# sergcpp/Ray

Measured on AMD Instinct MI355X. Metric: Msamples/sec (W*H*spp/time), higher is better.
Workload: dtype f32

## Files before the change

ray_amd/csrc/bvh_hooks.h:

```cpp
#pragma once

#include <string>
#include <vector>

#include "bvh4_build.h"
#include "lbvh.h"

namespace rayhip_bvh_hooks {

inline bool check_lbvh_args(const float *boxes, const uint32_t *groups, const uint32_t n_prims, const uint32_t n_groups, const uint32_t leaf_max,
                            std::string &why) {
    if (leaf_max < 1 || leaf_max > 8) {
        why = "leaf_max must be 1..8";
        return false;
    }
    if (n_prims >= 0x10000000u) {
        why = "too many primitives for a leaf word";
        return false;
    }
    if (n_prims && (!boxes || !groups)) {
        why = "null input";
        return false;
    }
    for (uint32_t p = 0; p < n_prims; ++p) {
        if (groups[p] >= n_groups) {
            why = "a group id is out of range";
            return false;
        }
    }
// ... 74 lines not shown
    }
    if (res.nodes.size() > n_nodes) {
        why = "more wide nodes than BVH2 nodes";
        return 1;
    }
    std::copy(res.nodes.begin(), res.nodes.end(), out_wide);
    std::copy(res.blas_root4.begin(), res.blas_root4.end(), out_roots4);
    *out_count = uint32_t(res.nodes.size());
    return 0;
}

RT_HD void test_node_item(const rt::Bvh4Node *wide, const uint32_t node, const float *o, const float *d, const float t, uint32_t *out_ref,
                          uint32_t *out_n_hit, float *out_dist) {
    const rt::f3 inv_d = rt::safe_invert(rt::f3{d[0], d[1], d[2]});
    uint32_t ref[4], n_hit;
    float dist[4];
    rt::bvh4_test_node(wide, node, rt::f3{o[0], o[1], o[2]}, inv_d, t, ref, n_hit, dist);
    for (int c = 0; c < 4; ++c) {
        out_ref[c] = ref[c], out_dist[c] = dist[c];
    }
    *out_n_hit = n_hit;
}

inline bool check_items(const uint32_t *node_index, const uint32_t n_items, const uint32_t n_wide, std::string &why) {
    for (uint32_t i = 0; i < n_items; ++i) {
        if (node_index[i] >= n_wide) {
            why = "an item names a node outside the array";
            return false;
        }
    }
    return true;
}

}
```

ray_amd/csrc/kernels_closest_refill.hip.h:

```cpp
#pragma once

#ifndef RT_REFILL_MIN
#define RT_REFILL_MIN 40
#endif
#ifndef RT_REFILL_MIN_WAVES
#define RT_REFILL_MIN_WAVES 6
#endif
#ifndef RT_REFILL_VOTE_NUM
#define RT_REFILL_VOTE_NUM 1
#define RT_REFILL_VOTE_DEN 1
#endif
#ifndef RT_REFILL_RUN
#define RT_REFILL_RUN 1
#endif
#ifndef RT_REFILL_MIN_DIRECT
#define RT_REFILL_MIN_DIRECT 40
#endif
template <int WIDE, int MIN_WAIT = RT_REFILL_MIN, bool DIRECT = false>
__global__ void __launch_bounds__(WAVE, RT_REFILL_MIN_WAVES) k_trace_closest_refill(const SceneView sc, const TraceParams tp, const RaySoA rays,
                                                               const HitSoA hits, const RayQueue queue, const int init_hits,
                                                               uint32_t *__restrict__ stack_spill, const Layering layers,
                                                               uint32_t *__restrict__ work ) {
    __shared__ uint32_t lds_stack[LDS_STACK_DEPTH * WAVE];
    const uint32_t lane = threadIdx.x;
#ifdef RT_PROFILE_TRACE
    if (threadIdx.x < 32) {
        s_prof_acc[threadIdx.x] = 0;
    }
    if (threadIdx.x == 0) {
        s_prof_last = __builtin_readcyclecounter();
    }
#endif
    LdsStack st;
    st.lane_base = &lds_stack[lane];
    st.spill_base = stack_spill + size_t(blockIdx.x) * size_t(STACK_SPILL_DEPTH * WAVE) + lane;
    st.size = 0;

    enum : uint32_t { IDLE = 0, TLAS = 1, BLAS = 2 };
#ifdef RT_PROFILE_TRACE
    uint32_t st_a = 0, st_b = 0, st_iter = 0, st_serv = 0, st_serv_lanes = 0, st_tlas = 0;
#endif
    uint32_t lvl = IDLE, slot = 0, cur = BVH4_SENTINEL, tos = BVH4_SENTINEL, size = 0, mi_index = 0, ray_flags = 0;
    uint32_t cur_bits = 0, tos_bits = 0, tri_base = 0, l0 = 0, l1 = 0, oct_inv = 0;
    bool res = false;
    f3 ro = {0.0f, 0.0f, 0.0f}, rd = {0.0f, 0.0f, 1.0f};
    f3 o = ro, d = rd, inv_d = rd;
    Hit h = make_hit();
    float t_val = 0.0f;
    uint32_t pool_slot = 0, pool_left = 0;
    ChunkWalk walk(queue.live_chunks(), work, RT_REFILL_RUN);

    auto begin_round = [&]() {
        t_val = h.t;
        res = false;
        size = 0;
        if (DIRECT) {
            tos = BVH4_SENTINEL;
            if ((sc.direct.ray_visibility & ray_flags) != 0) {
                o = transform_point(ro, sc.direct.inv_xform);
                d = transform_direction(rd, sc.direct.inv_xform);
                inv_d = safe_invert(d);
                st.write_at(size++, BVH4_SENTINEL);
                cur = sc.direct.root;
                lvl = (cur == BVH4_SENTINEL) ? TLAS : BLAS;
            } else {
                cur = BVH4_SENTINEL;
                lvl = TLAS;
            }
            return;
        }
        st.write_at(size++, BVH4_SENTINEL);
        tos = BVH4_SENTINEL;
        cur = tp.root_index;
        lvl = TLAS;
    };
    auto pop = [&]() {
        cur = tos;
        tos = st.read_at(--size);
    };
    auto leave_blas = [&]() {
        if (WIDE == 8) {
            if (lvl == BLAS && cur == BVH8_SENTINEL) {
                lvl = TLAS;
                cur = st.read_at(--size);
                tos = st.read_at(--size);
            }
        } else if (lvl == BLAS && cur == BVH4_SENTINEL) {
            lvl = TLAS;
            if (!DIRECT) {
                pop();
            }
        }
    };
    auto pop8 = [&]() {
        cur = tos, cur_bits = tos_bits;
        size -= 2;
        st.read2_at(size, tos, tos_bits);
    };

    uint32_t n_dead = 0;
    for (;;) {
        for (;;) {
            const bool in_blas = (lvl == BLAS);
            const bool leaf_word = (WIDE == 8 ? (l0 | l1) != 0u : (cur & BVH2_PRIM_COUNT_BITS) != 0);
            const unsigned long long m_blas = __builtin_amdgcn_ballot_w64(in_blas), m_leaf_word = __builtin_amdgcn_ballot_w64(leaf_word);
            const bool at_leaf = in_blas && leaf_word;
            const bool at_node = in_blas && !leaf_word;
            const int n_node = uniform_count(m_blas & ~m_leaf_word), n_leaf = uniform_count(m_blas & m_leaf_word);
            const int n_out = WAVE - n_node - n_leaf - int(n_dead);
#ifdef RT_PROFILE_TRACE
            st_a += n_node, st_b += n_leaf, st_iter += 1;
#endif
            if (n_node + n_leaf == 0 || n_out >= MIN_WAIT) {
                break;
            }
            if (n_node * RT_REFILL_VOTE_DEN >= n_leaf * RT_REFILL_VOTE_NUM) {
                if (at_node) {
                    if (WIDE == 8) {
                        const uint32_t node = bvh8_take_child(cur, cur_bits, oct_inv);
                        if ((cur_bits >> 8) != 0u) {
                            st.write2_at(size, tos, tos_bits);
                            size += 2;
                            tos = cur, tos_bits = cur_bits;
                        }
                        Bvh8Visit v;
                        bvh8_test_node(sc.nodes8, node, o, inv_d, h.t, oct_inv, v);
                        cur = v.child_base, cur_bits = v.bits, tri_base = v.tri_base, l0 = v.leaf[0], l1 = v.leaf[1];
                        if ((cur_bits >> 8) == 0u && (l0 | l1) == 0u) {
                            pop8();
                        }
                    } else {
                        bvh4_visit(sc.nodes4, o, inv_d, h.t, st, cur, tos, size);
                    }
                    leave_blas();
                }
                RT_PROF_T(19)
            } else {
                if (at_leaf) {
                    const uint32_t word = WIDE == 8 ? bvh8_take_leaf(tri_base, l0, l1) : cur;
                    const int tri_start = int(word & BVH2_PRIM_INDEX_BITS), tri_end = int(tri_start + ((word & BVH2_PRIM_COUNT_BITS) >> 29) + 1);
                    const bool hit = intersect_tris_closest(o, d, tri_table(sc), tri_start, tri_end, DIRECT ? int(sc.direct.mi) : int(mi_index), h);
                    res |= hit;
                    if (WIDE == 8) {
                        if ((l0 | l1) == 0u && (cur_bits >> 8) == 0u) {
                            pop8();
                        }
                    } else {
                        pop();
                    }
                    leave_blas();
                }
                RT_PROF_T(26)
            }
        }

#ifdef RT_PROFILE_TRACE
        st_serv += 1, st_serv_lanes += uint32_t(__popcll(__ballot(lvl != BLAS))) - n_dead;
#endif
        {
            const bool in_fin = (lvl == TLAS) && (cur == BVH4_SENTINEL);
            if (in_fin) {
                if (h.prim_index < 0) {
                    h.prim_index = -int(sc.tri_indices[-h.prim_index - 1]) - 1;
                } else {
                    h.prim_index = int(sc.tri_indices[h.prim_index]);
                }
                bool again = false;
                if (res && !hit_side_is_solid(sc, h)) {
                    const float4 cc = rays.c_cs[slot];
                    const uint2 xd = rays.xy_depth[slot];
                    Ray r;
                    r.c = {cc.x, cc.y, cc.z};
                    r.cone_spread = cc.w;
                    r.xy = xd.x, r.depth = xd.y;
                    const uint32_t xy_virtual = r.xy, layer = xy_layer(xy_virtual, layers);
                    TraceParams tpl = tp;
                    if (layer != 0) {
                        tpl.iteration = tp.iteration + int(layer);
                        tpl.rand_seed = layer_rand_seed(tpl.iteration);
                    }
// ... 141 lines not shown
```

ray_amd/csrc/kernels_shadow.hip.h:

```cpp
#pragma once

template <bool COUNT, int WIDE, int MINW = RT_TRACE_MIN_WAVES>
__global__ void __launch_bounds__(WAVE, MINW) k_trace_shadow(const SceneView sc, const TraceParams tp, const ShadowSoA shadow,
                                                      const RayQueue queue, const float limit,
                                                      const int img_w, float4 *__restrict__ temp_buf,
                                                      float4 *__restrict__ out_rc,
                                                      uint32_t *__restrict__ stack_spill,
                                                      unsigned long long *__restrict__ counters, const Layering layers) {
    __shared__ uint32_t lds_stack[LDS_STACK_DEPTH * WAVE];
    const uint32_t lane = threadIdx.x;
    const uint32_t n_live_chunks = queue.live_chunks();
    ChunkWalk walk(n_live_chunks);
    for (uint32_t c; walk.next(c);) {
        uint32_t stripe, slot0, n_live;
        if (!queue.chunk(c, stripe, slot0, n_live) || lane >= n_live) {
            continue;
        }
        const uint32_t i = slot0 + lane;
        const ShadowRay r = load_shadow(shadow, i);
        LdsStack st;
        st.lane_base = &lds_stack[lane];
        st.spill_base = stack_spill + size_t(blockIdx.x) * size_t(STACK_SPILL_DEPTH * WAVE) + lane;
        st.size = 0;
        TravCount tc = {0, 0, 0, 0, 0};
// ... 42 lines not shown
    st.size = 0;

    enum : uint32_t { IDLE = 0, TLAS = 1, BLAS = 2 };
    uint32_t lvl = IDLE, slot = 0, cur = BVH4_SENTINEL, tos = BVH4_SENTINEL, size = 0, mi_index = 0, crossed = 0;
    bool solid = false;
    f3 ro = {0.0f, 0.0f, 0.0f}, rd = {0.0f, 0.0f, 1.0f}, o = ro, d = rd, inv_d = rd;
    float dist = 0.0f;
    Hit h = make_hit();
    uint32_t pool_slot = 0, pool_left = 0;
    ChunkWalk walk(queue.live_chunks(), work, RT_SHADOW_RUN);

    auto begin_segment = [&]() {
        h = make_hit();
        h.t = dist;
        size = 0;
        if (DIRECT) {
            const bool walk_it = (sc.direct.ray_visibility & (1u << RAY_TYPE_SHADOW)) != 0 && sc.direct.root != BVH4_SENTINEL;
            o = transform_point(ro, sc.direct.inv_xform);
            d = transform_direction(rd, sc.direct.inv_xform);
            inv_d = safe_invert(d);
            st.write_at(size++, BVH4_SENTINEL);
            tos = BVH4_SENTINEL;
            cur = walk_it ? sc.direct.root : BVH4_SENTINEL;
            lvl = walk_it ? BLAS : TLAS;
            return;
        }
        st.write_at(size++, BVH4_SENTINEL);
        tos = BVH4_SENTINEL;
        cur = tp.root_index;
        lvl = TLAS;
    };
    auto pop = [&]() {
        cur = tos;
        tos = st.read_at(--size);
    };
    auto leave_blas = [&]() {
        if (lvl == BLAS && cur == BVH4_SENTINEL) {
            lvl = TLAS;
            if (!DIRECT) {
                pop();
            }
        }
    };
    auto deliver = [&](const f3 rc, const uint32_t xy_virtual) {
        if (out_rc) {
            out_rc[slot] = mkfloat4(rc.x, rc.y, rc.z, 0.0f);
        } else {
            add_shadow_pixel(rc, limit, xy_virtual, img_w, temp_buf);
        }
    };

    uint32_t n_dead = 0;
    for (;;) {
        for (;;) {
            const bool in_blas = (lvl == BLAS);
            const bool leaf_word = (cur & BVH2_PRIM_COUNT_BITS) != 0;
            const unsigned long long m_blas = __builtin_amdgcn_ballot_w64(in_blas), m_leaf_word = __builtin_amdgcn_ballot_w64(leaf_word);
            const bool at_leaf = in_blas && leaf_word;
            const bool at_node = in_blas && !leaf_word;
            const int n_node = uniform_count(m_blas & ~m_leaf_word), n_leaf = uniform_count(m_blas & m_leaf_word);
            const int n_out = WAVE - n_node - n_leaf - int(n_dead);
            if (n_node + n_leaf == 0 || n_out >= MIN_WAIT) {
                break;
            }
            if (n_node >= n_leaf) {
                if (at_node) {
                    bvh4_visit(sc.nodes4, o, inv_d, h.t, st, cur, tos, size);
                    leave_blas();
                }
            } else if (at_leaf) {
                const int tri_start = int(cur & BVH2_PRIM_INDEX_BITS), tri_end = int(tri_start + ((cur & BVH2_PRIM_COUNT_BITS) >> 29) + 1);
                bool stop = false;
                if (intersect_tris_any(o, d, tri_table(sc), sc.tri_materials, sc.tri_indices, tri_start, tri_end, DIRECT ? int(sc.direct.mi) : int(mi_index), h)) {
                    const bool is_backfacing = h.prim_index < 0;
                    const uint32_t prim = is_backfacing ? uint32_t(-h.prim_index - 1) : uint32_t(h.prim_index);
                    if (sc.all_solid != 0u) {
                        stop = true;
                    } else {
                        const rayhip_tri_mat_data md = sc.tri_materials[sc.tri_indices[prim]];
                        stop = (!is_backfacing && (md.front_mi & MATERIAL_SOLID_BIT)) || (is_backfacing && (md.back_mi & MATERIAL_SOLID_BIT));
                    }
                }
                if (stop) {
                    solid = true;
                    lvl = TLAS;
                    cur = BVH4_SENTINEL;
                } else {
                    pop();
                    leave_blas();
                }
            }
        }

        {
            const bool in_fin = (lvl == TLAS) && (cur == BVH4_SENTINEL);
            if (in_fin) {
                const uint32_t depth_word = float_as_uint(shadow.o_depth[slot].w);
                const float4 cx = shadow.c_xy[slot];
                const uint32_t xy_virtual = float_as_uint(cx.w);
                f3 rc = {cx.x, cx.y, cx.z};
                const bool over = (get_transp_depth(depth_word) + int(crossed)) > tp.max_transp_depth;
                if (solid || over) {
                    rc = {0.0f, 0.0f, 0.0f};
                }
                bool again = false;
                if (!solid && !over && h.v >= 0.0f) {
                    if (h.prim_index < 0) {
                        h.prim_index = -int(sc.tri_indices[-h.prim_index - 1]) - 1;
// ... 123 lines not shown
```

ray_amd/csrc/rayhip_hooks.hip.h:

```cpp
#pragma once


int rayhip_k_generate_primary_rays(rayhip_ctx *c, const rayhip_camera *cam, const int rect[4], int iteration,
                                   rayhip_ray *out_rays, rayhip_hit *out_hits, int *out_count) {
    if (use_device(c)) {
        return 1;
    }
    if (!c->w || !c->pmj.p || !c->filter_table.p) {
        return fail("k_generate_primary_rays needs resize + upload_static + set_filter_table first");
    }
    hipStream_t s = c->stream;
    const RayGenTiling tiling = make_raygen_tiling(c->w, c->h, rect[2], rect[3], c->shard);
    const size_t nslots = size_t(tiling.tiles) * 64u;
    if (c->clear_queues(1, s)) {
        return fail("queue counter clear failed");
    }
    const RayGenParams rg = make_raygen_params(*cam, c->w, c->h, rect, iteration, c->shard);
    k_raygen<<<grid_for(c, nslots, 256), 256, 0, s>>>(rg, c->sc.pmj, c->filter_table.as<float>(), c->px.required_samples,
                                                      c->rays[0], c->hits, c->ray_queue(0, nslots, 1), single_layer(c->w, c->h), tiling);
    HIP_TRY(hipGetLastError());
    uint32_t n = 0;
    HIP_TRY(hipMemcpyAsync(&n, c->ray_count(0), 4, hipMemcpyDeviceToHost, s));
    HIP_TRY(hipStreamSynchronize(s));
    HostRays hr;
// ... 261 lines not shown
    return 0;
}

__global__ void __launch_bounds__(256) k_bvh4_test_nodes(const Bvh4Node *__restrict__ wide, const uint32_t *__restrict__ node_index,
                                                        const float *__restrict__ ray_o, const float *__restrict__ ray_d,
                                                        const float *__restrict__ ray_t, const uint32_t n_items, uint32_t *__restrict__ out_ref,
                                                        uint32_t *__restrict__ out_n_hit, float *__restrict__ out_dist) {
    const uint32_t i = blockIdx.x * blockDim.x + threadIdx.x;
    if (i < n_items) {
        rayhip_bvh_hooks::test_node_item(wide, node_index[i], ray_o + size_t(i) * 3, ray_d + size_t(i) * 3, ray_t[i], out_ref + size_t(i) * 4,
                                         out_n_hit + i, out_dist + size_t(i) * 4);
    }
}

int rayhip_k_bvh4_test_nodes(rayhip_ctx *c, const void *wide, uint32_t n_wide, const uint32_t *node_index, const float *ray_o, const float *ray_d,
                             const float *ray_t, uint32_t n_items, uint32_t *out_ref, uint32_t *out_n_hit, float *out_dist) {
    if (use_device(c)) {
        return 1;
    }
    if (n_items == 0) {
        return 0;
    }
    std::string why;
    if (!rayhip_bvh_hooks::check_items(node_index, n_items, n_wide, why)) {
        return fail("k_bvh4_test_nodes: %s", why.c_str());
    }
    hipStream_t s = c->stream;
    const size_t n = n_items;
    DevBuf d_wide, d_idx, d_o, d_d, d_t, d_ref, d_hit, d_dist;
    if (d_wide.alloc(size_t(n_wide) * sizeof(Bvh4Node)) || d_idx.alloc(n * 4) || d_o.alloc(n * 12) || d_d.alloc(n * 12) || d_t.alloc(n * 4) ||
        d_ref.alloc(n * 16) || d_hit.alloc(n * 4) || d_dist.alloc(n * 16)) {
        return 1;
    }
    HIP_TRY(hipMemcpyAsync(d_wide.p, wide, size_t(n_wide) * sizeof(Bvh4Node), hipMemcpyHostToDevice, s));
    HIP_TRY(hipMemcpyAsync(d_idx.p, node_index, n * 4, hipMemcpyHostToDevice, s));
    HIP_TRY(hipMemcpyAsync(d_o.p, ray_o, n * 12, hipMemcpyHostToDevice, s));
    HIP_TRY(hipMemcpyAsync(d_d.p, ray_d, n * 12, hipMemcpyHostToDevice, s));
    HIP_TRY(hipMemcpyAsync(d_t.p, ray_t, n * 4, hipMemcpyHostToDevice, s));
    k_bvh4_test_nodes<<<(n_items + 255) / 256, 256, 0, s>>>(d_wide.as<Bvh4Node>(), d_idx.as<uint32_t>(), d_o.as<float>(), d_d.as<float>(),
                                                            d_t.as<float>(), n_items, d_ref.as<uint32_t>(), d_hit.as<uint32_t>(), d_dist.as<float>());
    HIP_TRY(hipGetLastError());
    HIP_TRY(hipMemcpyAsync(out_ref, d_ref.p, n * 16, hipMemcpyDeviceToHost, s));
    HIP_TRY(hipMemcpyAsync(out_n_hit, d_hit.p, n * 4, hipMemcpyDeviceToHost, s));
    HIP_TRY(hipMemcpyAsync(out_dist, d_dist.p, n * 16, hipMemcpyDeviceToHost, s));
    HIP_TRY(hipStreamSynchronize(s));
    d_wide.release(), d_idx.release(), d_o.release(), d_d.release(), d_t.release(), d_ref.release(), d_hit.release(), d_dist.release();
    return 0;
// ... 19 lines not shown
```

ray_amd/csrc/rayhip_upload.hip.h:

```cpp
#pragma once

static int upload_sky(rayhip_ctx *c, const rayhip_scene_desc *d) {
    c->sky_view = SkyView{};
    if (!(d->env.sky_map_spread_angle > 0.0f) || d->sky_count == 0) {
        return 0;
    }
    if (upload(c, c->sky_desc, d->sky, sizeof(rayhip_sky)) ||
        upload(c, c->sky_transmittance_lut, d->sky_transmittance_lut, size_t(d->sky_transmittance_lut_count) * sizeof(float)) ||
        upload(c, c->sky_multiscatter_lut, d->sky_multiscatter_lut, size_t(d->sky_multiscatter_lut_count) * sizeof(float)) ||
        upload(c, c->sky_dir_lights, d->sky_dir_lights, size_t(d->sky_dir_lights_count) * sizeof(uint32_t)) ||
        upload(c, c->sky_weather, d->sky_weather_tex, d->sky_weather_tex_count) || upload(c, c->sky_noise3d, d->sky_noise3d_tex, d->sky_noise3d_tex_count) ||
        upload(c, c->sky_curl, d->sky_curl_tex, d->sky_curl_tex_count) || upload(c, c->sky_moon, d->sky_moon_tex, d->sky_moon_tex_count) ||
        upload(c, c->sky_cirrus, d->sky_cirrus_tex, d->sky_cirrus_tex_count)) {
        return 1;
    }
    HIP_TRY(hipStreamSynchronize(c->stream));
    SkyView &v = c->sky_view;
    v.desc = c->sky_desc.as<rayhip_sky>();
    v.transmittance_lut = c->sky_transmittance_lut.as<float>(), v.multiscatter_lut = c->sky_multiscatter_lut.as<float>();
    v.dir_lights = c->sky_dir_lights.as<uint32_t>(), v.dir_lights_count = d->sky_dir_lights_count;
    v.weather = c->sky_weather.as<uint8_t>(), v.noise3d = c->sky_noise3d.as<uint8_t>(), v.curl = c->sky_curl.as<uint8_t>();
    v.moon = c->sky_moon.as<uint8_t>(), v.cirrus = c->sky_cirrus.as<uint8_t>();
    return 0;
}
// ... 392 lines not shown
        upload(c, c->tri_indices, tri_indices_in, n_tris * sizeof(uint32_t)) ||
        upload(c, c->mesh_instances, mis, size_t(d->mesh_instances_count) * sizeof(rayhip_mesh_instance))) {
        return 1;
    }
    c->instances_count = d->mesh_instances_count;
    if (pitch_tris(c, n_tris)) {
        return 1;
    }
    std::vector<uint32_t> blas_root4;
    size_t wide_bytes = 0;
    if (have8) {
        if (upload(c, c->nodes8, b8.nodes.data(), b8.nodes.size() * sizeof(Bvh8Node)) ||
            upload(c, c->blas_root4, b8.blas_root8.data(), b8.blas_root8.size() * sizeof(uint32_t))) {
            return 1;
        }
        wide = 8, blas_root4 = b8.blas_root8, wide_bytes = b8.nodes.size() * sizeof(Bvh8Node);
    } else if (want == 4 || want == 8) {
        if (collapse_bvh4(c, n2, n2_count, mis, d->mesh_instances_count, tlas_root, build_on_host, wide, blas_root4, wide_bytes)) {
            return 1;
        }
        trace(wide == 4 ? "bvh4 built" : "no wide BLAS");
    }
    HIP_TRY(hipStreamSynchronize(c->stream));
    c->trace.small_scene = wide != 0 && getenv("RAYHIP_NO_SMALL") == nullptr && wide_bytes + n_tris * sizeof(rayhip_tri_accel) <= (size_t(2) << 20);
    rayhip_update::collect_mesh_refs(n2, n2_count, mis, d->mesh_instances_count, tlas_root, wide ? blas_root4.data() : nullptr, c->mesh_refs);
    return prepare_refit(c, n2, n2_count, mis, d->mesh_instances_count, tlas_root, tri_indices_in, uint32_t(n_tris), d->vtx_indices, d->vtx_indices_count / 3,
                         d->vertices_count, have8);
}

static int upload_shading_arrays(rayhip_ctx *c, const rayhip_scene_desc *d, const bool all_sides_solid, const UploadTrace &trace) {
    UP(tri_materials)
    c->all_solid = all_sides_solid ? 1u : 0u;
    trace(all_sides_solid ? "every reachable triangle side is solid" : "some triangle sides are not solid");
    UP(materials)
    {
        bool refracts = false;
        for (uint32_t i = 0; i < d->materials_count; ++i) {
            const rayhip_material &m = d->materials[i];
            refracts |= m.type == NODE_REFRACTIVE || (m.type == NODE_PRINCIPLED && m.transmission_unorm != 0);
        }
        c->plain_ior = !refracts && !getenv("RAYHIP_NO_PLAIN_IOR");
        trace(refracts ? "refractive surfaces: rays carry their ior stacks" : "no refractive surface: the ior plane of the rays is not used");
    }
    UP(vertices)
    UP(vtx_indices)
    const uint32_t n_tris = d->vtx_indices_count / 3;
    if (c->tri_verts.alloc(size_t(n_tris) * TRI_VERTS_STRIDE * sizeof(float4)) ||
        c->tri_bitangents.alloc(size_t(n_tris) * TRI_BITANGENTS_STRIDE * sizeof(float4))) {
        return 1;
    }
    if (n_tris) {
        k_fill_tri_verts<<<(n_tris + 255) / 256, 256, 0, c->stream>>>(c->vertices.as<rayhip_vertex>(), d->vertices_count,
                                                                      c->vtx_indices.as<uint32_t>(), n_tris,
                                                                      c->tri_materials.as<rayhip_tri_mat_data>(), d->tri_materials_count,
                                                                      c->tri_verts.as<float4>(), c->tri_bitangents.as<float4>());
        HIP_TRY(hipGetLastError());
    }
    return 0;
}

static int upload_textures_and_env(rayhip_ctx *c, const rayhip_scene_desc *d) {
// ... 31 lines not shown
        std::string why;
        if (!rayhip_validate::validate(*d, why, &all_sides_solid, &materials_used)) {
            return fail("%s", why.c_str());
        }
    }
    trace("validated");
    const bool build_on_host = getenv("RAYHIP_BVH_BUILD_ON_HOST") != nullptr && atoi(getenv("RAYHIP_BVH_BUILD_ON_HOST")) != 0;
    rayhip_rebuild::Rebuilt rebuilt;
    rayhip_scene_desc d_rebuilt = *d;
    if (refine_trees(c, d, build_on_host, trace, rebuilt, d_rebuilt)) {
        return 1;
    }
    if (rebuilt.ok) {
        d = &d_rebuilt;
    }
    rayhip_layout::Result lay = layout_pass(d, rebuilt.ok);
    trace(lay.applied ? "layout applied" : lay.why_not);
    int wide = 0;
    uint32_t tlas_root = 0xffffffffu;
    if (upload_bottom_level(c, d, lay, build_on_host, trace, wide, tlas_root)) {
        return 1;
    }
    trace("bvh uploaded");
    if (upload_shading_arrays(c, d, all_sides_solid, trace)) {
        return 1;
    }
    trace("tri_verts done");
    if (upload_lights(c, d)) {
        return 1;
    }
    keep_light_vertices(c, d);
    if (upload_vertex_checks(c, true) || upload_instance_checks(c, d) || upload_material_checks(c, d, &materials_used)) {
        return 1;
    }
    trace("lights done");
    if (upload_textures_and_env(c, d)) {
        return 1;
    }
    c->wide = wide;
    c->geometry = {d->vertices_count, d->vtx_indices_count, d->tri_materials_count, d->materials_count};
    rayhip_lbvh::Box root_box = rayhip_lbvh::empty_box();
    if (d->tlas_root != 0xffffffffu && d->tlas_root < d->nodes_count) {
        root_box = rayhip_rebuild::node_box(d->nodes[d->tlas_root]);
    }
    if (upload_sky(c, d)) {
        return 1;
    }
// ... 273 lines not shown
```

ray_amd/csrc/rt_bvh4.h:

```cpp
#pragma once

#include "rt_isect.h"

namespace rt {


#ifndef RT_BVH4_PINNED_FETCH
#define RT_BVH4_PINNED_FETCH 1
#endif

struct alignas(16) Bvh4Node {
    float org[3];
    float step_x;
    uint32_t child[4];
    uint32_t qlo[3];
    uint32_t qhi[3];
    float step_y, step_z;
};
static_assert(sizeof(Bvh4Node) == 64, "Bvh4Node must be one 64-byte fetch unit");

constexpr uint32_t BVH4_SENTINEL = 0x1fffffffu;
constexpr uint32_t BVH4_EMPTY = 0xffffffffu;
static_assert(BVH4_SENTINEL + 1u == (BVH2_PRIM_COUNT_BITS & (0u - BVH2_PRIM_COUNT_BITS)), "the sentinel is the largest word without a count bit");

RT_HD float bvh4_dequant(const uint32_t q, const float scale, const float org) { return __builtin_fmaf(float(q), scale, org); }

RT_HD void bvh4_test_node(const Bvh4Node *nodes4, const uint32_t cur, const f3 ro, const f3 inv_d, const float t, uint32_t ref[4],
                          uint32_t &n_hit, float *out_dist = nullptr) {
    RT_PROF_T(16)
    RT_PROF_LANES(0)
    const float4 *np = reinterpret_cast<const float4 *>(nodes4 + cur);
#if defined(__HIP_DEVICE_COMPILE__) && RT_BVH4_PINNED_FETCH
    float4 w0, w1, w2, w3;
    asm volatile("global_load_dwordx4 %0, %4, off\n\tglobal_load_dwordx4 %1, %4, off offset:16\n\tglobal_load_dwordx4 %2, %4, off offset:32\n\t"
                 "global_load_dwordx4 %3, %4, off offset:48\n\ts_waitcnt vmcnt(0)"
                 : "=&v"(w0), "=&v"(w1), "=&v"(w2), "=&v"(w3)
                 : "v"(np)
                 : "memory");
#else
    const float4 w0 = np[0], w1 = np[1], w2 = np[2], w3 = np[3];
#endif
    RT_PROF_WAIT(w0, w1, w2, w3)
    RT_PROF_T(17)
    const float step[3] = {w0.w, w3.z, w3.w};
    const uint32_t child[4] = {float_as_uint(w1.x), float_as_uint(w1.y), float_as_uint(w1.z), float_as_uint(w1.w)};

    const float org[3] = {w0.x, w0.y, w0.z}, o[3] = {ro.x, ro.y, ro.z}, id[3] = {inv_d.x, inv_d.y, inv_d.z};
    const uint32_t qlo_w[3] = {float_as_uint(w2.x), float_as_uint(w2.y), float_as_uint(w2.z)};
    const uint32_t qhi_w[3] = {float_as_uint(w2.w), float_as_uint(w3.x), float_as_uint(w3.y)};
    float k[3], base_in[3], base_out[3];
    uint32_t q_in[3], q_out[3];
    for (int a = 0; a < 3; ++a) {
        k[a] = step[a] * id[a];
        const float base = (org[a] - o[a]) * id[a];
        const float err = __builtin_fmaf(255.0f, fabsf(k[a]), fabsf(base)) * 9.5367431640625e-07f;
        base_in[a] = base - err, base_out[a] = base + err;
        const bool forward = id[a] >= 0.0f;
        q_in[a] = forward ? qlo_w[a] : qhi_w[a], q_out[a] = forward ? qhi_w[a] : qlo_w[a];
    }

    const float none = 3.402823466e+38f;
    float dist[4];
    n_hit = 0;
    for (int c = 0; c < 4; ++c) {
        const int sh = 8 * c;
        float t_in[3], t_out[3];
        for (int a = 0; a < 3; ++a) {
            t_in[a] = __builtin_fmaf(float((q_in[a] >> sh) & 0xffu), k[a], base_in[a]);
            t_out[a] = __builtin_fmaf(float((q_out[a] >> sh) & 0xffu), k[a], base_out[a]);
        }
        const float tmin = fmaxf(fmaxf(fmaxf(t_in[0], t_in[1]), t_in[2]), 0.0f), tmax = fminf(fminf(fminf(t_out[0], t_out[1]), t_out[2]), t);
        const bool hit = tmin <= tmax && child[c] != BVH4_EMPTY;
        dist[c] = hit ? tmin : none;
        ref[c] = child[c];
        n_hit += hit ? 1u : 0u;
    }
#define RT_CSWAP(a, b)                                                                                                  \
    {                                                                                                                   \
        const bool sw = dist[b] < dist[a];                                                                              \
        const float da = sw ? dist[b] : dist[a], db = sw ? dist[a] : dist[b];                                           \
        const uint32_t ra = sw ? ref[b] : ref[a], rb = sw ? ref[a] : ref[b];                                            \
        dist[a] = da, dist[b] = db, ref[a] = ra, ref[b] = rb;                                                           \
    }
    RT_CSWAP(0, 1)
    RT_CSWAP(2, 3)
    RT_CSWAP(0, 2)
    RT_CSWAP(1, 3)
    RT_CSWAP(1, 2)
#undef RT_CSWAP
    if (out_dist) {
        for (int c = 0; c < 4; ++c) {
            out_dist[c] = dist[c];
        }
    }
    RT_PROF_T(18)
// ... 154 lines not shown
```

ray_amd/csrc/rt_isect.h:

```cpp
#pragma once

#include "rt_rng.h"
#include "rt_texture.h"
#include "rt_types.h"

namespace rt {

struct ArrayStack {
    uint32_t data[4 * MAX_STACK_SIZE];
    uint32_t size = 0;
    RT_HD void push(uint32_t v) { data[size++] = v; }
    RT_HD uint32_t pop() { return data[--size]; }
    RT_HD bool fast_range(uint32_t) const { return true; }
    RT_HD void write_at(uint32_t idx, uint32_t v) { data[idx] = v; }
    RT_HD void write3_fast(uint32_t idx, uint32_t a, uint32_t b, uint32_t c) { data[idx] = a, data[idx + 1] = b, data[idx + 2] = c; }
    RT_HD uint32_t read_at(uint32_t idx) const { return data[idx]; }
    RT_HD void write2_at(uint32_t idx, uint32_t a, uint32_t b) { data[idx] = a, data[idx + 1] = b; }
    RT_HD void read2_at(uint32_t idx, uint32_t &a, uint32_t &b) const { a = data[idx], b = data[idx + 1]; }
};

#define RT_SIGN_OF(f) (((f) >= 0) ? 1 : -1)

struct TriData {
    float4 n, u, v;
};
struct TriTable {
    const float4 *rows;
    uint32_t pitch;
};
RT_HD TriData load_tri(const TriTable tris, const uint32_t i) {
    const float4 *p = tris.rows + size_t(i) * tris.pitch;
    TriData t;
    t.n = p[0], t.u = p[1], t.v = p[2];
    return t;
}

RT_HD void intersect_tri(const f3 ro, const f3 rd, const TriData &tri, const uint32_t prim_index, Hit &inter) {
    const float det = rd.x * tri.n.x + rd.y * tri.n.y + rd.z * tri.n.z;
    const float dett = tri.n.w - (ro.x * tri.n.x + ro.y * tri.n.y + ro.z * tri.n.z);
    bool ok = !(det == 0.0f || RT_SIGN_OF(dett) != RT_SIGN_OF(det * inter.t - dett));

    const float p0 = det * ro.x + dett * rd.x, p1 = det * ro.y + dett * rd.y, p2 = det * ro.z + dett * rd.z;

    const float detu = (p0 * tri.u.x + p1 * tri.u.y + p2 * tri.u.z) + det * tri.u.w;
    ok = ok && !(RT_SIGN_OF(detu) != RT_SIGN_OF(det - detu));

    const float detv = (p0 * tri.v.x + p1 * tri.v.y + p2 * tri.v.z) + det * tri.v.w;
    ok = ok && !(RT_SIGN_OF(detv) != RT_SIGN_OF(det - detu - detv));

    if (ok) {
        const float rdet = (1.0f / det);
        inter.prim_index = (det < 0.0f) ? int(prim_index) : -int(prim_index) - 1;
        inter.t = dett * rdet;
        inter.u = detu * rdet;
        inter.v = detv * rdet;
    }
}
#undef RT_SIGN_OF

RT_HD bool bbox_test(const f3 o, const f3 inv_d, const float t, const float mn[3], const float mx[3], float &out_dist) {
    const float lo_x = inv_d.x * (mn[0] - o.x), hi_x = inv_d.x * (mx[0] - o.x);
    const float lo_y = inv_d.y * (mn[1] - o.y), hi_y = inv_d.y * (mx[1] - o.y);
    const float lo_z = inv_d.z * (mn[2] - o.z), hi_z = inv_d.z * (mx[2] - o.z);

    const float tmin = fmaxf(fmaxf(fminf(lo_x, hi_x), fminf(lo_y, hi_y)), fminf(lo_z, hi_z));
    float tmax = fminf(fminf(fmaxf(lo_x, hi_x), fmaxf(lo_y, hi_y)), fmaxf(lo_z, hi_z));
    tmax *= 1.00000024f;

    out_dist = tmin;
    return tmin <= tmax && tmin <= t && tmax > 0;
}

}
```

ray_amd/csrc/rt_traverse.h:

```cpp
#pragma once

#include "rt_bvh4.h"
#include "rt_bvh8.h"
#include "rt_isect.h"

namespace rt {

template <class Stack>
RT_HD void bvh2_node_step(const rayhip_bvh2_node *nodes, const f3 ro, const f3 inv_d, const float t, uint32_t &cur,
                          Stack &st, TravCount *cnt) {
    const float4 *np = reinterpret_cast<const float4 *>(nodes + cur);
    const float4 d0 = np[0], d1 = np[1], d2 = np[2], links = np[3];
    const uint32_t left_child = float_as_uint(links.x), right_child = float_as_uint(links.y);
    if (cnt) {
        ++cnt->nodes;
        cnt->max_stack = st.size > cnt->max_stack ? st.size : cnt->max_stack;
    }
    const float ch0_min[3] = {d0.x, d0.z, d2.x};
    const float ch0_max[3] = {d0.y, d0.w, d2.y};
    const float ch1_min[3] = {d1.x, d1.z, d2.z};
    const float ch1_max[3] = {d1.y, d1.w, d2.w};

    float ch0_dist, ch1_dist;
    const bool ch0_res = bbox_test(ro, inv_d, t, ch0_min, ch0_max, ch0_dist);
// ... 34 lines not shown
                break;
            }
        }

        while ((leaf_node & BVH2_PRIM_COUNT_BITS) != 0) {
            if (leaf(leaf_node)) {
                st.size = base;
                return true;
            }
            leaf_node = cur;
            if ((cur & BVH2_PRIM_COUNT_BITS) != 0) {
                cur = st.pop();
            }
        }
    }
    st.size = base;
    return false;
}

RT_HD TriTable tri_table(const SceneView &sc) { return TriTable{reinterpret_cast<const float4 *>(sc.tris), sc.tri_pitch}; }

RT_HD bool intersect_tris_closest(const f3 ro, const f3 rd, const TriTable tris, const int tri_start,
                                  const int tri_end, const int obj_index, Hit &out_inter) {
    Hit inter;
    inter.obj_index = obj_index;
    inter.prim_index = 0;
    inter.t = out_inter.t;
    inter.u = 0.0f;
    inter.v = -1.0f;
    RT_PROF_T(20)
    const TriData tri0 = load_tri(tris, uint32_t(tri_start)), tri1 = load_tri(tris, uint32_t(tri_start + 1));
    RT_PROF_WAIT(tri0.n, tri0.u, tri1.n, tri1.v)
    RT_PROF_T(21)
    RT_PROF_LANES(2)
    intersect_tri(ro, rd, tri0, uint32_t(tri_start), inter);
    RT_PROF_LANES(2)
    intersect_tri(ro, rd, tri1, uint32_t(tri_start + 1), inter);
    for (int i = tri_start + 2; i < tri_end; ++i) {
        RT_PROF_LANES(2)
        const TriData tri = load_tri(tris, uint32_t(i));
        intersect_tri(ro, rd, tri, uint32_t(i), inter);
    }
    RT_PROF_T(22)
    const bool hit = inter.v >= 0.0f;
    out_inter.obj_index = hit ? inter.obj_index : out_inter.obj_index;
    out_inter.prim_index = hit ? inter.prim_index : out_inter.prim_index;
    out_inter.t = inter.t;
    out_inter.u = hit ? inter.u : out_inter.u;
    out_inter.v = hit ? inter.v : out_inter.v;
    return hit;
}

RT_HD bool intersect_tris_any(const f3 ro, const f3 rd, const TriTable tris,
                              const rayhip_tri_mat_data *materials, const uint32_t *indices, const int tri_start,
                              const int tri_end, const int obj_index, Hit &out_inter) {
    Hit inter;
    inter.obj_index = obj_index;
    inter.prim_index = 0;
    inter.t = out_inter.t;
    inter.u = 0.0f;
    inter.v = -1.0f;
    const auto solid_hit = [&](const int i) {
        return inter.v >= 0.0f && ((inter.prim_index > 0 && (materials[indices[i]].front_mi & MATERIAL_SOLID_BIT)) ||
                                   (inter.prim_index < 0 && (materials[indices[i]].back_mi & MATERIAL_SOLID_BIT)));
    };
    const TriData tri0 = load_tri(tris, uint32_t(tri_start)), tri1 = load_tri(tris, uint32_t(tri_start + 1));
    intersect_tri(ro, rd, tri0, uint32_t(tri_start), inter);
    if (!solid_hit(tri_start)) {
        intersect_tri(ro, rd, tri1, uint32_t(tri_start + 1), inter);
        if (!solid_hit(tri_start + 1)) {
            for (int i = tri_start + 2; i < tri_end; ++i) {
                const TriData tri = load_tri(tris, uint32_t(i));
                intersect_tri(ro, rd, tri, uint32_t(i), inter);
                if (solid_hit(i)) {
                    break;
                }
            }
        }
    }
    const bool hit = inter.v >= 0.0f;
    out_inter.obj_index = hit ? inter.obj_index : out_inter.obj_index;
    out_inter.prim_index = hit ? inter.prim_index : out_inter.prim_index;
    out_inter.t = inter.t;
    out_inter.u = hit ? inter.u : out_inter.u;
    out_inter.v = hit ? inter.v : out_inter.v;
    return hit;
}

template <int WIDE = 0, class Stack>
RT_HD bool traverse_closest(const SceneView &sc, const f3 ro, const f3 rd, const uint32_t ray_flags,
                            const uint32_t root_index, Hit &inter, Stack &st, TravCount *cnt) {
    bool res = false;
    const f3 inv_d = safe_invert(rd);

    walk_bvh2(sc.nodes, root_index, ro, inv_d, inter.t, st, cnt, [&](const uint32_t leaf_node) {
        const uint32_t mi_index = (leaf_node & BVH2_PRIM_INDEX_BITS);
        const rayhip_mesh_instance &mi = sc.mesh_instances[mi_index];
        if ((mi.ray_visibility & ray_flags) != 0) {
            if (cnt) {
                ++cnt->instances;
            }
            const f3 _ro = transform_point(ro, mi.inv_xform);
            const f3 _rd = transform_direction(rd, mi.inv_xform);
            const f3 _inv_d = safe_invert(_rd);
            RT_PROF_T(23)
            RT_PROF_LANES(4)
            auto blas_leaf_fn = [&](const uint32_t blas_leaf) {
                const int tri_start = int(blas_leaf & BVH2_PRIM_INDEX_BITS),
// ... 299 lines not shown
```

ray_amd/csrc/trace_select.h:

```cpp
#pragma once

#include <stdint.h>

#include "../../include/rayhip.h"

namespace rt {

struct TraceConfig {
    int refill_waves = 0;
    int refill_resident = 0;
    int refill_resident4 = 0;
    bool refill_secondary_only = false;
    bool refill_primary_whole = false;
    bool refill_pool = false;
    int pool_waves = 0, pool_resident = 0;
    bool pool_scene = false;
    bool shadow_refill = true;
    int shadow_resident = 0;
    int tune_primary_waves = 0, tune_shadow_waves = 5;
    bool small_scene = false;
    bool direct_entry = true;
    bool direct_scene = false;
    bool overlap_shadow = true;
};

inline void set_refill_mode(TraceConfig &t, const int mode) {
    t.refill_secondary_only = mode == 2 || mode == 3 || mode == 4;
    t.refill_primary_whole = mode == 3 || mode == 4;
    t.refill_pool = mode == 4;
}

enum class ClosestForm {
    Counted8, Counted4, Counted0,
    Plain8, Plain8Small, Plain4, Plain4Small, Plain0,
    Whole8, Whole4, Whole4Direct,
    Lane8, Lane4, Lane4Direct,
    Pooled,
};
enum class ShadowForm {
    Counted8, Counted4, Counted0,
    Plain8, Plain8Small, Plain4, Plain4Small, Plain0,
    Refill, RefillDirect,
};

enum class TraceRole { Primary, Secondary, Hook };

inline bool is_whole(ClosestForm f) { return f == ClosestForm::Whole8 || f == ClosestForm::Whole4 || f == ClosestForm::Whole4Direct; }
// ... 72 lines not shown
```

Baseline: 806.8.

## Trim traversal overhead: 32-bit node offsets, direct-mode level logic, in-place triangle hits

Several micro-optimizations to the BVH traversal kernels. Node and triangle fetches now use 32-bit byte offsets added to a scalar base, which allows SGPR-base plus VGPR-offset global loads. The direct-scene refill kernels drop the TLAS/BLAS level ballot and treat every lane as being in the BLAS. The empty-slot check is skipped for child slots 0 and 1, and triangle intersection writes straight into the output hit instead of a temporary. Host checks enforce the 4 GB offset limit and the slot invariant, and the refraction scan now skips materials that are not used.

```diff
diff --git a/ray_amd/csrc/bvh_hooks.h b/ray_amd/csrc/bvh_hooks.h
--- a/ray_amd/csrc/bvh_hooks.h
+++ b/ray_amd/csrc/bvh_hooks.h
@@ -5,6 +5,7 @@
 
 #include "bvh4_build.h"
 #include "lbvh.h"
+#include "trace_select.h"
 
 namespace rayhip_bvh_hooks {
 
@@ -125,6 +126,20 @@
     *out_n_hit = n_hit;
 }
 
+inline bool check_wide_nodes(const rt::Bvh4Node *wide, const uint32_t n_wide, std::string &why) {
+    if (!rt::walk_offsets_fit(uint64_t(n_wide) * sizeof(rt::Bvh4Node), 0)) {
+        why = "the wide nodes reach 4 GB (the node test addresses them by 32-bit offsets)";
+        return false;
+    }
+    for (uint32_t n = 0; n < n_wide; ++n) {
+        if (!rt::bvh4_slots_ok(wide[n].child)) {
+            why = "wide node " + std::to_string(n) + " has an empty child slot 0 or 1 (only slots 2 and 3 may be empty)";
+            return false;
+        }
+    }
+    return true;
+}
+
 inline bool check_items(const uint32_t *node_index, const uint32_t n_items, const uint32_t n_wide, std::string &why) {
     for (uint32_t i = 0; i < n_items; ++i) {
         if (node_index[i] >= n_wide) {
diff --git a/ray_amd/csrc/kernels_closest_refill.hip.h b/ray_amd/csrc/kernels_closest_refill.hip.h
--- a/ray_amd/csrc/kernels_closest_refill.hip.h
+++ b/ray_amd/csrc/kernels_closest_refill.hip.h
@@ -21,6 +21,7 @@
                                                                const HitSoA hits, const RayQueue queue, const int init_hits,
                                                                uint32_t *__restrict__ stack_spill, const Layering layers,
                                                                uint32_t *__restrict__ work ) {
+    static_assert(!DIRECT || WIDE == 4, "direct entry walks the 4-wide tree");
     __shared__ uint32_t lds_stack[LDS_STACK_DEPTH * WAVE];
     const uint32_t lane = threadIdx.x;
 #ifdef RT_PROFILE_TRACE
@@ -62,11 +63,10 @@
                 inv_d = safe_invert(d);
                 st.write_at(size++, BVH4_SENTINEL);
                 cur = sc.direct.root;
-                lvl = (cur == BVH4_SENTINEL) ? TLAS : BLAS;
             } else {
                 cur = BVH4_SENTINEL;
-                lvl = TLAS;
-            }
+            }
+            lvl = TLAS;
             return;
         }
         st.write_at(size++, BVH4_SENTINEL);
@@ -85,11 +85,9 @@
                 cur = st.read_at(--size);
                 tos = st.read_at(--size);
             }
-        } else if (lvl == BLAS && cur == BVH4_SENTINEL) {
+        } else if (!DIRECT && lvl == BLAS && cur == BVH4_SENTINEL) {
             lvl = TLAS;
-            if (!DIRECT) {
-                pop();
-            }
+            pop();
         }
     };
     auto pop8 = [&]() {
@@ -99,14 +97,18 @@
     };
 
     uint32_t n_dead = 0;
+    const Bvh4Node *nodes4 = sc.nodes4;
+    asm volatile("" : "+s"(nodes4));
     for (;;) {
         for (;;) {
-            const bool in_blas = (lvl == BLAS);
-            const bool leaf_word = (WIDE == 8 ? (l0 | l1) != 0u : (cur & BVH2_PRIM_COUNT_BITS) != 0);
-            const unsigned long long m_blas = __builtin_amdgcn_ballot_w64(in_blas), m_leaf_word = __builtin_amdgcn_ballot_w64(leaf_word);
+            const bool in_blas = DIRECT || (lvl == BLAS);
+            const bool leaf_word = DIRECT ? cur > BVH4_SENTINEL : (WIDE == 8 ? (l0 | l1) != 0u : (cur & BVH2_PRIM_COUNT_BITS) != 0);
+            const bool node_word = cur < BVH4_SENTINEL;
+            const unsigned long long m_blas = DIRECT ? 0ull : __builtin_amdgcn_ballot_w64(in_blas), m_leaf_word = __builtin_amdgcn_ballot_w64(leaf_word);
             const bool at_leaf = in_blas && leaf_word;
-            const bool at_node = in_blas && !leaf_word;
-            const int n_node = uniform_count(m_blas & ~m_leaf_word), n_leaf = uniform_count(m_blas & m_leaf_word);
+            const bool at_node = DIRECT ? node_word : in_blas && !leaf_word;
+            const int n_node = uniform_count(DIRECT ? __builtin_amdgcn_ballot_w64(node_word) : m_blas & ~m_leaf_word),
+                      n_leaf = uniform_count(DIRECT ? m_leaf_word : m_blas & m_leaf_word);
             const int n_out = WAVE - n_node - n_leaf - int(n_dead);
 #ifdef RT_PROFILE_TRACE
             st_a += n_node, st_b += n_leaf, st_iter += 1;
@@ -130,7 +132,7 @@
                             pop8();
                         }
                     } else {
-                        bvh4_visit(sc.nodes4, o, inv_d, h.t, st, cur, tos, size);
+                        bvh4_visit(nodes4, o, inv_d, h.t, st, cur, tos, size);
                     }
                     leave_blas();
                 }
@@ -155,7 +157,7 @@
         }
 
 #ifdef RT_PROFILE_TRACE
-        st_serv += 1, st_serv_lanes += uint32_t(__popcll(__ballot(lvl != BLAS))) - n_dead;
+        st_serv += 1, st_serv_lanes += uint32_t(__popcll(__ballot(DIRECT ? cur == BVH4_SENTINEL : lvl != BLAS))) - n_dead;
 #endif
         {
             const bool in_fin = (lvl == TLAS) && (cur == BVH4_SENTINEL);
diff --git a/ray_amd/csrc/kernels_shadow.hip.h b/ray_amd/csrc/kernels_shadow.hip.h
--- a/ray_amd/csrc/kernels_shadow.hip.h
+++ b/ray_amd/csrc/kernels_shadow.hip.h
@@ -88,7 +88,7 @@
             st.write_at(size++, BVH4_SENTINEL);
             tos = BVH4_SENTINEL;
             cur = walk_it ? sc.direct.root : BVH4_SENTINEL;
-            lvl = walk_it ? BLAS : TLAS;
+            lvl = TLAS;
             return;
         }
         st.write_at(size++, BVH4_SENTINEL);
@@ -101,11 +101,9 @@
         tos = st.read_at(--size);
     };
     auto leave_blas = [&]() {
-        if (lvl == BLAS && cur == BVH4_SENTINEL) {
+        if (!DIRECT && lvl == BLAS && cur == BVH4_SENTINEL) {
             lvl = TLAS;
-            if (!DIRECT) {
-                pop();
-            }
+            pop();
         }
     };
     auto deliver = [&](const f3 rc, const uint32_t xy_virtual) {
@@ -119,12 +117,14 @@
     uint32_t n_dead = 0;
     for (;;) {
         for (;;) {
-            const bool in_blas = (lvl == BLAS);
-            const bool leaf_word = (cur & BVH2_PRIM_COUNT_BITS) != 0;
-            const unsigned long long m_blas = __builtin_amdgcn_ballot_w64(in_blas), m_leaf_word = __builtin_amdgcn_ballot_w64(leaf_word);
+            const bool in_blas = DIRECT || (lvl == BLAS);
+            const bool leaf_word = DIRECT ? cur > BVH4_SENTINEL : (cur & BVH2_PRIM_COUNT_BITS) != 0;
+            const bool node_word = cur < BVH4_SENTINEL;
+            const unsigned long long m_blas = DIRECT ? 0ull : __builtin_amdgcn_ballot_w64(in_blas), m_leaf_word = __builtin_amdgcn_ballot_w64(leaf_word);
             const bool at_leaf = in_blas && leaf_word;
-            const bool at_node = in_blas && !leaf_word;
-            const int n_node = uniform_count(m_blas & ~m_leaf_word), n_leaf = uniform_count(m_blas & m_leaf_word);
+            const bool at_node = DIRECT ? node_word : in_blas && !leaf_word;
+            const int n_node = uniform_count(DIRECT ? __builtin_amdgcn_ballot_w64(node_word) : m_blas & ~m_leaf_word),
+                      n_leaf = uniform_count(DIRECT ? m_leaf_word : m_blas & m_leaf_word);
             const int n_out = WAVE - n_node - n_leaf - int(n_dead);
             if (n_node + n_leaf == 0 || n_out >= MIN_WAIT) {
                 break;
@@ -149,7 +149,9 @@
                 }
                 if (stop) {
                     solid = true;
-                    lvl = TLAS;
+                    if (!DIRECT) {
+                        lvl = TLAS;
+                    }
                     cur = BVH4_SENTINEL;
                 } else {
                     pop();
diff --git a/ray_amd/csrc/rayhip_hooks.hip.h b/ray_amd/csrc/rayhip_hooks.hip.h
--- a/ray_amd/csrc/rayhip_hooks.hip.h
+++ b/ray_amd/csrc/rayhip_hooks.hip.h
@@ -307,7 +307,7 @@
         return 0;
     }
     std::string why;
-    if (!rayhip_bvh_hooks::check_items(node_index, n_items, n_wide, why)) {
+    if (!rayhip_bvh_hooks::check_items(node_index, n_items, n_wide, why) || !rayhip_bvh_hooks::check_wide_nodes(static_cast<const Bvh4Node *>(wide), n_wide, why)) {
         return fail("k_bvh4_test_nodes: %s", why.c_str());
     }
     hipStream_t s = c->stream;
diff --git a/ray_amd/csrc/rayhip_upload.hip.h b/ray_amd/csrc/rayhip_upload.hip.h
--- a/ray_amd/csrc/rayhip_upload.hip.h
+++ b/ray_amd/csrc/rayhip_upload.hip.h
@@ -438,21 +438,30 @@
         trace(wide == 4 ? "bvh4 built" : "no wide BLAS");
     }
     HIP_TRY(hipStreamSynchronize(c->stream));
+    if (!walk_offsets_fit(wide == 4 ? uint64_t(wide_bytes) : 0u, uint64_t(n_tris) * c->tri_pitch * 16u)) {
+        return fail("the scene's 4-wide nodes (%llu bytes) or triangle records (%llu bytes) reach 4 GB: the traversal kernels address both by 32-bit offsets",
+                    (unsigned long long)(wide == 4 ? wide_bytes : 0), (unsigned long long)(uint64_t(n_tris) * c->tri_pitch * 16u));
+    }
     c->trace.small_scene = wide != 0 && getenv("RAYHIP_NO_SMALL") == nullptr && wide_bytes + n_tris * sizeof(rayhip_tri_accel) <= (size_t(2) << 20);
     rayhip_update::collect_mesh_refs(n2, n2_count, mis, d->mesh_instances_count, tlas_root, wide ? blas_root4.data() : nullptr, c->mesh_refs);
     return prepare_refit(c, n2, n2_count, mis, d->mesh_instances_count, tlas_root, tri_indices_in, uint32_t(n_tris), d->vtx_indices, d->vtx_indices_count / 3,
                          d->vertices_count, have8);
 }
 
-static int upload_shading_arrays(rayhip_ctx *c, const rayhip_scene_desc *d, const bool all_sides_solid, const UploadTrace &trace) {
+static int upload_shading_arrays(rayhip_ctx *c, const rayhip_scene_desc *d, const bool all_sides_solid, const std::vector<uint8_t> &materials_used,
+                                 const UploadTrace &trace) {
     UP(tri_materials)
     c->all_solid = all_sides_solid ? 1u : 0u;
     trace(all_sides_solid ? "every reachable triangle side is solid" : "some triangle sides are not solid");
     UP(materials)
     {
         bool refracts = false;
+        const bool know_used = materials_used.size() == d->materials_count;
         for (uint32_t i = 0; i < d->materials_count; ++i) {
             const rayhip_material &m = d->materials[i];
+            if (know_used && !materials_used[i]) {
+                continue;
+            }
             refracts |= m.type == NODE_REFRACTIVE || (m.type == NODE_PRINCIPLED && m.transmission_unorm != 0);
         }
         c->plain_ior = !refracts && !getenv("RAYHIP_NO_PLAIN_IOR");
@@ -530,7 +539,7 @@
         return 1;
     }
     trace("bvh uploaded");
-    if (upload_shading_arrays(c, d, all_sides_solid, trace)) {
+    if (upload_shading_arrays(c, d, all_sides_solid, materials_used, trace)) {
         return 1;
     }
     trace("tri_verts done");
diff --git a/ray_amd/csrc/rt_bvh4.h b/ray_amd/csrc/rt_bvh4.h
--- a/ray_amd/csrc/rt_bvh4.h
+++ b/ray_amd/csrc/rt_bvh4.h
@@ -21,6 +21,9 @@
 
 constexpr uint32_t BVH4_SENTINEL = 0x1fffffffu;
 constexpr uint32_t BVH4_EMPTY = 0xffffffffu;
+RT_HD bool bvh4_slots_ok(const uint32_t child[4]) {
+    return child[0] != BVH4_EMPTY && child[1] != BVH4_EMPTY;
+}
 static_assert(BVH4_SENTINEL + 1u == (BVH2_PRIM_COUNT_BITS & (0u - BVH2_PRIM_COUNT_BITS)), "the sentinel is the largest word without a count bit");
 
 RT_HD float bvh4_dequant(const uint32_t q, const float scale, const float org) { return __builtin_fmaf(float(q), scale, org); }
@@ -29,15 +32,23 @@
                           uint32_t &n_hit, float *out_dist = nullptr) {
     RT_PROF_T(16)
     RT_PROF_LANES(0)
-    const float4 *np = reinterpret_cast<const float4 *>(nodes4 + cur);
+#if defined(__HIP_DEVICE_COMPILE__)
+    const uint32_t node_off = cur << 6;
+    static_assert(sizeof(Bvh4Node) == 1u << 6, "node_off is the byte offset of a node");
+#endif
 #if defined(__HIP_DEVICE_COMPILE__) && RT_BVH4_PINNED_FETCH
     float4 w0, w1, w2, w3;
-    asm volatile("global_load_dwordx4 %0, %4, off\n\tglobal_load_dwordx4 %1, %4, off offset:16\n\tglobal_load_dwordx4 %2, %4, off offset:32\n\t"
-                 "global_load_dwordx4 %3, %4, off offset:48\n\ts_waitcnt vmcnt(0)"
+    asm volatile("s_nop 4\n\tglobal_load_dwordx4 %0, %4, %5\n\tglobal_load_dwordx4 %1, %4, %5 offset:16\n\tglobal_load_dwordx4 %2, %4, %5 offset:32\n\t"
+                 "global_load_dwordx4 %3, %4, %5 offset:48\n\ts_waitcnt vmcnt(0)"
                  : "=&v"(w0), "=&v"(w1), "=&v"(w2), "=&v"(w3)
-                 : "v"(np)
+                 : "v"(node_off), "s"(nodes4)
                  : "memory");
 #else
+#if defined(__HIP_DEVICE_COMPILE__)
+    const float4 *np = reinterpret_cast<const float4 *>(reinterpret_cast<const char *>(nodes4) + node_off);
+#else
+    const float4 *np = reinterpret_cast<const float4 *>(nodes4 + cur);
+#endif
     const float4 w0 = np[0], w1 = np[1], w2 = np[2], w3 = np[3];
 #endif
     RT_PROF_WAIT(w0, w1, w2, w3)
@@ -70,7 +81,7 @@
             t_out[a] = __builtin_fmaf(float((q_out[a] >> sh) & 0xffu), k[a], base_out[a]);
         }
         const float tmin = fmaxf(fmaxf(fmaxf(t_in[0], t_in[1]), t_in[2]), 0.0f), tmax = fminf(fminf(fminf(t_out[0], t_out[1]), t_out[2]), t);
-        const bool hit = tmin <= tmax && child[c] != BVH4_EMPTY;
+        const bool hit = tmin <= tmax && (c < 2 || child[c] != BVH4_EMPTY);
         dist[c] = hit ? tmin : none;
         ref[c] = child[c];
         n_hit += hit ? 1u : 0u;
diff --git a/ray_amd/csrc/rt_isect.h b/ray_amd/csrc/rt_isect.h
--- a/ray_amd/csrc/rt_isect.h
+++ b/ray_amd/csrc/rt_isect.h
@@ -29,13 +29,17 @@
     uint32_t pitch;
 };
 RT_HD TriData load_tri(const TriTable tris, const uint32_t i) {
+#if defined(__HIP_DEVICE_COMPILE__)
+    const float4 *p = reinterpret_cast<const float4 *>(reinterpret_cast<const char *>(tris.rows) + i * (tris.pitch * 16u));
+#else
     const float4 *p = tris.rows + size_t(i) * tris.pitch;
+#endif
     TriData t;
     t.n = p[0], t.u = p[1], t.v = p[2];
     return t;
 }
 
-RT_HD void intersect_tri(const f3 ro, const f3 rd, const TriData &tri, const uint32_t prim_index, Hit &inter) {
+RT_HD void intersect_tri(const f3 ro, const f3 rd, const TriData &tri, const uint32_t prim_index, const int obj_index, Hit &inter, bool &hit) {
     const float det = rd.x * tri.n.x + rd.y * tri.n.y + rd.z * tri.n.z;
     const float dett = tri.n.w - (ro.x * tri.n.x + ro.y * tri.n.y + ro.z * tri.n.z);
     bool ok = !(det == 0.0f || RT_SIGN_OF(dett) != RT_SIGN_OF(det * inter.t - dett));
@@ -50,6 +54,8 @@
 
     if (ok) {
         const float rdet = (1.0f / det);
+        hit = true;
+        inter.obj_index = obj_index;
         inter.prim_index = (det < 0.0f) ? int(prim_index) : -int(prim_index) - 1;
         inter.t = dett * rdet;
         inter.u = detu * rdet;
diff --git a/ray_amd/csrc/rt_traverse.h b/ray_amd/csrc/rt_traverse.h
--- a/ray_amd/csrc/rt_traverse.h
+++ b/ray_amd/csrc/rt_traverse.h
@@ -80,68 +80,46 @@
 
 RT_HD bool intersect_tris_closest(const f3 ro, const f3 rd, const TriTable tris, const int tri_start,
                                   const int tri_end, const int obj_index, Hit &out_inter) {
-    Hit inter;
-    inter.obj_index = obj_index;
-    inter.prim_index = 0;
-    inter.t = out_inter.t;
-    inter.u = 0.0f;
-    inter.v = -1.0f;
+    bool hit = false;
     RT_PROF_T(20)
     const TriData tri0 = load_tri(tris, uint32_t(tri_start)), tri1 = load_tri(tris, uint32_t(tri_start + 1));
     RT_PROF_WAIT(tri0.n, tri0.u, tri1.n, tri1.v)
     RT_PROF_T(21)
     RT_PROF_LANES(2)
-    intersect_tri(ro, rd, tri0, uint32_t(tri_start), inter);
+    intersect_tri(ro, rd, tri0, uint32_t(tri_start), obj_index, out_inter, hit);
     RT_PROF_LANES(2)
-    intersect_tri(ro, rd, tri1, uint32_t(tri_start + 1), inter);
+    intersect_tri(ro, rd, tri1, uint32_t(tri_start + 1), obj_index, out_inter, hit);
     for (int i = tri_start + 2; i < tri_end; ++i) {
         RT_PROF_LANES(2)
         const TriData tri = load_tri(tris, uint32_t(i));
-        intersect_tri(ro, rd, tri, uint32_t(i), inter);
+        intersect_tri(ro, rd, tri, uint32_t(i), obj_index, out_inter, hit);
     }
     RT_PROF_T(22)
-    const bool hit = inter.v >= 0.0f;
-    out_inter.obj_index = hit ? inter.obj_index : out_inter.obj_index;
-    out_inter.prim_index = hit ? inter.prim_index : out_inter.prim_index;
-    out_inter.t = inter.t;
-    out_inter.u = hit ? inter.u : out_inter.u;
-    out_inter.v = hit ? inter.v : out_inter.v;
     return hit;
 }
 
 RT_HD bool intersect_tris_any(const f3 ro, const f3 rd, const TriTable tris,
                               const rayhip_tri_mat_data *materials, const uint32_t *indices, const int tri_start,
                               const int tri_end, const int obj_index, Hit &out_inter) {
-    Hit inter;
-    inter.obj_index = obj_index;
-    inter.prim_index = 0;
-    inter.t = out_inter.t;
-    inter.u = 0.0f;
-    inter.v = -1.0f;
+    bool hit = false;
     const auto solid_hit = [&](const int i) {
-        return inter.v >= 0.0f && ((inter.prim_index > 0 && (materials[indices[i]].front_mi & MATERIAL_SOLID_BIT)) ||
-                                   (inter.prim_index < 0 && (materials[indices[i]].back_mi & MATERIAL_SOLID_BIT)));
+        return hit && ((out_inter.prim_index > 0 && (materials[indices[i]].front_mi & MATERIAL_SOLID_BIT)) ||
+                       (out_inter.prim_index < 0 && (materials[indices[i]].back_mi & MATERIAL_SOLID_BIT)));
     };
     const TriData tri0 = load_tri(tris, uint32_t(tri_start)), tri1 = load_tri(tris, uint32_t(tri_start + 1));
-    intersect_tri(ro, rd, tri0, uint32_t(tri_start), inter);
+    intersect_tri(ro, rd, tri0, uint32_t(tri_start), obj_index, out_inter, hit);
     if (!solid_hit(tri_start)) {
-        intersect_tri(ro, rd, tri1, uint32_t(tri_start + 1), inter);
+        intersect_tri(ro, rd, tri1, uint32_t(tri_start + 1), obj_index, out_inter, hit);
         if (!solid_hit(tri_start + 1)) {
             for (int i = tri_start + 2; i < tri_end; ++i) {
                 const TriData tri = load_tri(tris, uint32_t(i));
-                intersect_tri(ro, rd, tri, uint32_t(i), inter);
+                intersect_tri(ro, rd, tri, uint32_t(i), obj_index, out_inter, hit);
                 if (solid_hit(i)) {
                     break;
                 }
             }
         }
     }
-    const bool hit = inter.v >= 0.0f;
-    out_inter.obj_index = hit ? inter.obj_index : out_inter.obj_index;
-    out_inter.prim_index = hit ? inter.prim_index : out_inter.prim_index;
-    out_inter.t = inter.t;
-    out_inter.u = hit ? inter.u : out_inter.u;
-    out_inter.v = hit ? inter.v : out_inter.v;
     return hit;
 }
 
diff --git a/ray_amd/csrc/trace_select.h b/ray_amd/csrc/trace_select.h
--- a/ray_amd/csrc/trace_select.h
+++ b/ray_amd/csrc/trace_select.h
@@ -23,6 +23,11 @@
     bool direct_scene = false;
     bool overlap_shadow = true;
 };
+
+inline bool walk_offsets_fit(const uint64_t nodes4_bytes, const uint64_t tri_table_bytes) {
+    constexpr uint64_t LIMIT = uint64_t(1) << 32;
+    return nodes4_bytes < LIMIT && tri_table_bytes < LIMIT;
+}
 
 inline void set_refill_mode(TraceConfig &t, const int mode) {
     t.refill_secondary_only = mode == 2 || mode == 3 || mode == 4;
```

After: 814.4 (median of 6 runs). No clear change (+0.9%).
